# temudschin/xfemm

Measured on AMD Instinct MI355X. Metric: solved DoF/s (assembly+CG to tol) on 2M-tri magnetostatic, higher is better.
Workload: dtype f64; 1 GPU; configs[2]: synthetic 2000000-tri square-domain magnetostatic, linear mu, tol 1e-08; triangles=2000000, dof_total=1002001, dof_per_gpu=1002001, nnz=7006001, pcg_iters=18, newton_iters=1, pcg=Chronopoulos-Gear + AMG V-cycle, parallelism=single GPU

## Files before the change

### include/xfemm_kernels.h

```cpp
#ifndef XFEMM_KERNELS_H
#define XFEMM_KERNELS_H

#ifdef __cplusplus
extern "C" {
#endif

enum {
    XFK_OK = 0,
    XFK_ERR_ARG = -1,
    XFK_ERR_HIP = -2,
    XFK_ERR_SINGULAR = -3,
    XFK_ERR_NOCONV = -4,
    XFK_ERR_UNSUPPORTED = -5
};

typedef struct {
    double mu_x, mu_y;
    double H_c;
    double J_re;
    double Cduct;
    double LamFill;
    int LamType;
    int BHpoints;
    const double *B;
// ... 386 lines not shown
typedef struct {
    int sweeps;
    double theta, omega;
    int dense_max, fold, col16, f32, wlevel;
} xfk_amg_probe_opts;
typedef struct {
    int n, nc, fold, has16, has32, w_at;
    long long nnz, pnnz, fnnz;
    double weight, rho_f;
} xfk_amg_level_info;
typedef struct {
    int levels, dense_coarse, cinv_f64, traced;
    xfk_amg_level_info level[16];
} xfk_amg_info;
enum { XFK_AMG_A = 0, XFK_AMG_P = 1, XFK_AMG_R = 2, XFK_AMG_PF = 3, XFK_AMG_RF = 4,
       XFK_AMG_PLAIN_COLS = 16, XFK_AMG_F64_VALS = 32 };
enum { XFK_AMG_DINV = 0, XFK_AMG_DENSE = 1 };
enum { XFK_AMG_TR_SFLAG = 0, XFK_AMG_TR_SDEG = 1, XFK_AMG_TR_AGG = 2, XFK_AMG_TR_AGG_PRE = 3,
       XFK_AMG_TR_ROOT = 4, XFK_AMG_TR_DFINV = 5, XFK_AMG_TR_WF = 6 };
int xfk_amg_probe_create(int n, const int *rowptr, const int *col, const double *val, int device,
                         const xfk_amg_probe_opts *opts, int trace, xfk_amg_probe **out);
int xfk_amg_probe_info(xfk_amg_probe *probe, xfk_amg_info *info);
int xfk_amg_probe_level_size(xfk_amg_probe *probe, int level, int sel, int *rows, int *cols, long long *nnz);
int xfk_amg_probe_level_csr(xfk_amg_probe *probe, int level, int sel, int *rowptr, int *col, double *val);
int xfk_amg_probe_tiles(xfk_amg_probe *probe, int sel, int *tiles, int *wide);
int xfk_amg_probe_vector(xfk_amg_probe *probe, int level, int what, double *out);
int xfk_amg_probe_trace(xfk_amg_probe *probe, int level, int what, void *out);
int xfk_amg_probe_apply(xfk_amg_probe *probe, int nvec, const double *R, double *U);
int xfk_amg_probe_refresh(xfk_amg_probe *probe, const double *val, int fold);
void xfk_amg_probe_destroy(xfk_amg_probe *probe);

int xfk_get_csr(xfk_problem *prob, int *rowptr, int *col, double *val, double *b);
long long xfk_get_nnz(xfk_problem *prob);
double xfk_spmv_col_bytes(xfk_problem *prob);
int xfk_get_stream(xfk_problem *prob, void **hip_stream);

int xfk_pcg_solve_csr(int n, const int *rowptr, const int *col, const double *val,
                      const double *b, double *V, int flag, double precision,
                      int device, long long *iters, double *er);
int xfk_pcg_solve_csr_pc(int n, const int *rowptr, const int *col, const double *val,
                         const double *b, double *V, int flag, double precision,
                         int device, int precond, long long *iters, double *er);

int xfk_age_element_matrix(double ci, double co, double K, double Ki, double *MG);

int xfk_pcg_time(xfk_problem *prob, int iters, double *ms_spmv, double *ms_iter);

typedef struct {
    char name[64];
    int calls;
    double ms_total;
    double bytes_per_call;
} xfk_phase;
enum { XFK_PROFILE_SETUP = 1 };
int xfk_phase_profile(xfk_problem *prob, int iters, int flags, xfk_phase *out, int cap, int *count);

int xfk_alloc_stats(double *out4, int reset);

int xfk_problem_memory(const xfk_problem *prob, long long *out4);
int xfk_cache_stats(long long *out3);
int xfk_release_cache(void);

int xfk_amg_forget_hints(void);

int xfk_sort_elements(int n_elems, const unsigned *score, int device, int *perm);

// ... 14 lines not shown
```

### xfemm_amd/csrc/xfk_api.hip

```cpp
#include <hipcub/hipcub.hpp>

#include "xfk_amg.h"
#include "xfk_spmv.h"

#include <algorithm>
#include <atomic>
#include <chrono>
#include <cmath>
#include <cstring>
#include <map>
#include <mutex>
#include <iterator>
#include <set>
#include <type_traits>
#include <unordered_map>

#include "xfk_age.h"
#include "xfk_comm.h"
#include "xfk_kernels.h"
#include "xfk_magdir.h"
#include <cstdio>
#include <cstdlib>
#include "xfk_partition.h"

// ... 722 lines not shown
    launch_row_build(s, N, P->p_raw.p, P->n2e_ptr.p, P->n2e.p, fp, fc, T.rowtmp, T.rowcnt, P->n2e.p);
    XFK_CHECK(exclusive_scan(P, T.rowcnt, P->rowptr.p, N));
    XFK_CHECK(hipMemcpyAsync(P->hpin, P->rowptr.p + N, sizeof(int), hipMemcpyDeviceToHost, s));
    XFK_CHECK(hipMemcpyAsync(P->hpin + 1, P->rowptr.p + P->N, sizeof(int), hipMemcpyDeviceToHost, s));
    P->hpin[5] = 0;
    if (!P->harmonic && N > 0 && P->amg && P->amg->cap_hint.empty()) {
        void *tmp = nullptr;
        size_t bytes = 0;
        XFK_CHECK(hipcub::DeviceReduce::Max(tmp, bytes, T.rowcnt, T.cnt + 3, N, s));
        XFK_CHECK(cub_scratch(P, bytes, &tmp));
        XFK_CHECK(hipcub::DeviceReduce::Max(tmp, bytes, T.rowcnt, T.cnt + 3, N, s));
        XFK_CHECK(hipMemcpyAsync(P->hpin + 5, T.cnt + 3, sizeof(int), hipMemcpyDeviceToHost, s));
    }
    const long long bound_nnz = 6LL * NE + N + nfill;
    const bool defer = !P->harmonic && P->age_key.empty() && P->pbc_entry_key.empty() &&
                       bound_nnz * 12 <= (512LL << 20);
    long long cap_nnz;
    if (defer) {
        if (!P->nnz_ev) XFK_CHECK(hipEventCreateWithFlags(&P->nnz_ev, hipEventDisableTiming));
        XFK_CHECK(hipEventRecord(P->nnz_ev, s));
        P->nnz_pending = true;
        cap_nnz = bound_nnz;
    } else {
        XFK_CHECK(hipStreamSynchronize(s));
        P->nnz = P->hpin[0];
        P->nnz_own = P->hpin[1];
        P->row_max = P->hpin[5];
        P->nnz_pending = false;
        cap_nnz = P->nnz;
    }
    XFK_CHECK(P->col.alloc(cap_nnz));
    XFK_CHECK(P->val.alloc(cap_nnz));
    XFK_CHECK(P->diag.alloc(N));
    launch_row_copy(s, N, P->p_raw.p, P->n2e_ptr.p, P->n2e.p, fp, fc, T.rowtmp, P->rowptr.p, P->col.p, P->diag.p);

    P->ncolors = 0;
    P->color_rounds = 0;
    if (P->harmonic) {
    XFK_CHECK(P->color.alloc(NE));
    XFK_CHECK(hipMemsetAsync(P->color.p, 0xff, sizeof(int) * NE, s));
    constexpr int kSyncRounds = 6;
    XFK_CHECK(hipMemsetAsync(T.active, 1, (size_t)NL, s));
    int round = 0, last = 0;
    for (;;) {
        XFK_REQUIRE(round < SymTmp::kMaxRounds, XFK_ERR_UNSUPPORTED, "element colouring did not terminate");
        for (int k = 0; k < kSyncRounds; ++k, ++round)
            launch_jp_round(s, NL, NE, round, T.active, T.cnt + 2, P->p_raw.p, P->n2e_ptr.p, P->n2e.p, P->color.p,
                            T.maxkey, T.used);
        XFK_CHECK(d2h(&last, T.cnt + 2, sizeof(int), s));
        if (last < round) break;
    }
    round = last + 1;
    P->color_rounds = round;
    const int maxc = SymTmp::kMaxColors;
    launch_color_hist(s, NE, P->color.p, T.hist, maxc);
    std::vector<int> hh(maxc + 1);
    XFK_CHECK(d2h(hh.data(), T.hist, sizeof(int) * (maxc + 1), s));
    XFK_REQUIRE(hh[maxc] == 0, XFK_ERR_UNSUPPORTED, "more than 128 element colours needed");
    int nc = 0;
    for (int c = 0; c < maxc; ++c)
        if (hh[c]) nc = c + 1;
    P->ncolors = nc;
    P->color_off.assign(nc + 1, 0);
    for (int c = 0; c < nc; ++c) P->color_off[c + 1] = P->color_off[c] + hh[c];

    XFK_CHECK(P->perm.alloc(NE));
    launch_iota(s, NE, T.iota);
    {
        void *tmp = nullptr;
        size_t bytes = 0;
        XFK_CHECK(hipcub::DeviceRadixSort::SortPairs(tmp, bytes, P->color.p, T.keys_out, T.iota, P->perm.p, NE, 0,
                                                     8, s));
        XFK_CHECK(cub_scratch(P, bytes, &tmp));
        XFK_CHECK(hipcub::DeviceRadixSort::SortPairs(tmp, bytes, P->color.p, T.keys_out, T.iota, P->perm.p, NE, 0,
                                                     8, s));
    }
    XFK_CHECK(P->erec.alloc(NE));
    XFK_CHECK(P->ebits.alloc(NE));
    XFK_CHECK(P->slot.alloc(9 * (size_t)NE));
    launch_build_erec(s, NE, P->perm.p, P->p_raw.p, P->lbl_raw.p, P->ebits_raw.p, P->erec.p, P->ebits.p, T.iperm);
    launch_build_slots(s, NE, N, P->p_raw.p, T.iperm, P->rowptr.p, P->col.p, P->slot.p, T.cnt);
    }

    launch_mark_fix_adj(s, N, P->rowptr.p, P->col.p, P->fixed.p, T.flag);
    XFK_CHECK(P->fix_cols_row.alloc(N));
    launch_compact_flags(s, N, T.flag, T.cnt + 1, P->fix_cols_row.p);
    if (P->harmonic) {
        XFK_CHECK(hipMemcpyAsync(P->hpin + 2, T.cnt, sizeof(int) * 2, hipMemcpyDeviceToHost, s));
        XFK_CHECK(hipStreamSynchronize(s));
        const int hc[2] = {P->hpin[2], P->hpin[3]};
        XFK_REQUIRE(hc[0] == 0, XFK_ERR_HIP, "internal: element slot missing from the CSR pattern");
        P->nfix_cols = hc[1];
    } else {
        XFK_CHECK(P->nfix_dev.alloc(1));
        XFK_CHECK(hipMemcpyAsync(P->nfix_dev.p, T.cnt + 1, sizeof(int), hipMemcpyDeviceToDevice, s));
        P->nfix_cols = -1;
    }
    XFK_CHECK(P->mu1.alloc(NE));
    XFK_CHECK(P->mu2.alloc(NE));
    if (!P->harmonic) {
        XFK_CHECK(P->mu1b.alloc(NE));
        XFK_CHECK(P->mu2b.alloc(NE));
        if (P->any_nonlinear && !P->axi) {
            XFK_CHECK(P->dv_el.alloc(NE));
            XFK_CHECK(P->on_el.alloc(NE));
        }
        XFK_CHECK(P->asm_miss.alloc(1));
        XFK_CHECK(hipMemsetAsync(P->asm_miss.p, 0, sizeof(int), s));
        P->miss_checked = false;
    }

    P->age_n = 0;
    if (!P->age_key.empty()) {
        std::vector<int> rc;
        std::vector<double> v;
        for (size_t m = 0; m < P->age_key.size(); ++m) {
            const int r = (int)(P->age_key[m] >> 32), c = (int)(P->age_key[m] & 0xffffffff);
            rc.push_back(r); rc.push_back(c); v.push_back(P->age_val[m]);
            if (r != c) { rc.push_back(c); rc.push_back(r); v.push_back(P->age_val[m]); }
        }
        const int na = (int)v.size();
        DBuf<int> d_rc;
        XFK_CHECK(upload(d_rc, rc.data(), rc.size(), s));
        XFK_CHECK(upload(P->age_v, v.data(), v.size(), s));
        XFK_CHECK(P->age_slot.alloc(na));
        launch_lookup_slots(s, na, d_rc.p, P->rowptr.p, P->col.p, P->age_slot.p);
        std::vector<int> chk(na);
        XFK_CHECK(d2h(chk.data(), P->age_slot.p, sizeof(int) * na, s));
// ... 127 lines not shown
    A.blocks = P->blocks.p;
    A.lines = P->lines.p;
    A.circs = P->circs.p;
    A.bhB = P->bhB.p;
    A.bhH = P->bhH.p;
    A.bhS = P->bhS.p;
    A.mu1 = P->mu1.p;
    A.mu2 = P->mu2.p;
    A.V = P->V.p;
    A.val = P->val.p;
    A.b = P->b.p;
    A.iter = iter;
    A.axi = P->axi ? 1 : 0;
    A.ext_ro = P->ext_ro;
    A.ext_ri = P->ext_ri;
    A.ext_zo = P->ext_zo;
    A.p_raw = P->p_raw.p;
    A.lbl_raw = P->lbl_raw.p;
    A.ebits_raw = P->ebits_raw.p;
    A.n2e_ptr = P->n2e_ptr.p;
    A.n2e = P->n2e.p;
    A.rowptr = P->rowptr.p;
    A.col = P->col.p;
    A.mu1_out = P->any_nonlinear ? P->mu1b.p : nullptr;
    A.mu2_out = P->any_nonlinear ? P->mu2b.p : nullptr;
    A.miss = P->asm_miss.p;
    const bool pre = P->any_nonlinear && !P->axi && P->dv_el.p && env_int("XFK_ASM_STATE", 1) != 0;
    A.dv_el = pre ? P->dv_el.p : nullptr;
    A.on_el = pre ? P->on_el.p : nullptr;
    A.n_el = P->NE;
    if (P->electro) launch_electro_rows(s, P);
    else if (P->heat) launch_heat_rows(s, P);
    else if (P->mask) launch_mask_rows(s, P);
    else launch_assemble_rows(s, P->NR, A);
    std::swap(P->mu1.p, P->mu1b.p);
    std::swap(P->mu1.n, P->mu1b.n);
    std::swap(P->mu2.p, P->mu2b.p);
    std::swap(P->mu2.n, P->mu2b.n);
    launch_add_at_slots(s, P->age_n, P->age_slot.p, P->age_v.p, P->val.p);
    launch_point_currents(s, P->npt, P->pt_nodes.p, P->pt_J.p, P->b.p);
    launch_dirichlet(s, P->nfix_rows, P->fix_rows.p, P->nfix_cols, P->nfix_dev.p, P->N, P->fix_cols_row.p,
                     P->rowptr.p, P->col.p, P->diag.p, P->fixed.p, P->fix_first.p, P->fix_last.p, P->val.p, P->b.p);
    launch_map(s, P->pm_n, P->pm_dst.p, P->pm_ptr.p, P->pm_src.p, P->pm_w.p, P->val.p, P->pm_tmp.p);
    launch_map(s, P->pb_n, P->pb_dst.p, P->pb_ptr.p, P->pb_src.p, P->pb_w.p, P->b.p, P->pb_tmp.p);
    XFK_CHECK(hipGetLastError());
    return XFK_OK;
}

static int alloc_cg(xfk_problem *P)
{
    const int N = P->N, NL = P->NL;
    int G = std::max(cg_grid(N), cg_axpy_grid(N));
    if (P->comm)
        for (int q = 0; q < P->nranks; ++q) {
            const int nq = (int)(row_begin(P->N_global, q + 1, P->nranks) - row_begin(P->N_global, q, P->nranks));
            G = std::max(G, std::max(cg_grid(nq), cg_axpy_grid(nq)));
        }
    P->Gpart = G;
    XFK_CHECK(P->R2.alloc((size_t)N));
    XFK_CHECK(P->W2.alloc((size_t)N));
    XFK_CHECK(P->Z2.alloc((size_t)N + NL));
    XFK_CHECK(P->part_loc.alloc(4 * (size_t)G));
    if (P->comm) {
        XFK_CHECK(P->part_glob_buf.alloc(4 * (size_t)G));
        P->part_glob = P->part_glob_buf.p;
    } else {
// ... 1530 lines not shown
    return XFK_OK;
}

long long xfk_get_nnz(xfk_problem *P) { return P && xfk_resolve_nnz(P) == XFK_OK ? P->nnz_own : -1; }

double xfk_spmv_col_bytes(xfk_problem *P)
{
    if (!P || xfk_resolve_nnz(P) != XFK_OK) return -1.0;
    const unsigned short *c16;
    const int *cbase;
    spmv_col16(P, c16, cbase);
    if (!c16 || P->nnz_own <= 0) return 4.0;
    const int N = P->N, nt = (N + kCgBlock - 1) / kCgBlock;
    std::vector<int> base(nt), rp(N + 1);
    if (d2h(base.data(), cbase, sizeof(int) * nt, P->stream) != hipSuccess ||
        d2h(rp.data(), P->rowptr.p, sizeof(int) * (N + 1), P->stream) != hipSuccess)
        return -1.0;
    long long wide = 0;
    for (int t = 0; t < nt; ++t)
        if (base[t] == kNoColBase) wide += rp[std::min(N, (t + 1) * kCgBlock)] - rp[t * kCgBlock];
    return (2.0 * (double)P->nnz_own + 2.0 * (double)wide) / (double)P->nnz_own;
}

int xfk_get_csr(xfk_problem *P, int *rowptr, int *col, double *val, double *b)
{
    XFK_REQUIRE(P && P->symbolic_ready, XFK_ERR_ARG, "no assembled system");
    XFK_CHECK(hipSetDevice(P->device));
    XFK_CHECK(hipStreamSynchronize(P->stream));
    if (xfk_resolve_nnz(P) != XFK_OK) return XFK_ERR_HIP;
    if (rowptr) XFK_CHECK(d2h(rowptr, P->rowptr.p, sizeof(int) * (P->N + 1), P->stream));
    if (col) XFK_CHECK(d2h(col, P->col.p, sizeof(int) * P->nnz_own, P->stream));
    if (val) XFK_CHECK(d2h(val, P->val.p, sizeof(double) * P->nnz_own, P->stream));
    if (b) XFK_CHECK(d2h(b, P->b.p, sizeof(double) * P->N, P->stream));
    return XFK_OK;
}

int xfk_get_stream(xfk_problem *P, void **st)
{
    XFK_REQUIRE(P && st, XFK_ERR_ARG, "null argument");
    *st = (void *)P->stream;
    return XFK_OK;
}

int xfk_pcg_solve_csr(int n, const int *rowptr, const int *col, const double *val, const double *b, double *V,
                      int flag, double precision, int device, long long *iters, double *er)
{
    return xfk_pcg_solve_csr_pc(n, rowptr, col, val, b, V, flag, precision, device, XFK_PRECOND_JACOBI, iters, er);
}

int xfk_set_option(xfk_problem *P, int option, double value)
{
    XFK_REQUIRE(P, XFK_ERR_ARG, "null problem");
    switch (option) {
    case XFK_OPT_PRECOND:
        XFK_REQUIRE(value == XFK_PRECOND_JACOBI || value == XFK_PRECOND_AMG, XFK_ERR_ARG, "unknown preconditioner");
        P->precond = (int)value;
        return XFK_OK;
    case XFK_OPT_AMG_SWEEPS:
        XFK_REQUIRE(value >= 1 && value <= 8 && value == (int)value, XFK_ERR_ARG, "AMG sweeps must be 1..8");
        P->amg_sweeps = (int)value;
        return XFK_OK;
    case XFK_OPT_AMG_THETA:
        XFK_REQUIRE(value >= 0.0 && value < 1.0, XFK_ERR_ARG, "AMG strength threshold must be in [0, 1)");
        P->amg_theta = value;
        return XFK_OK;
    case XFK_OPT_AMG_OMEGA:
// ... 360 lines not shown
```

### xfemm_amd/csrc/xfk_device.hip

```cpp
#include "xfk_kernels.h"
#include "xfk_axi.h"
#include "xfk_spmv.h"

namespace xfk {


__device__ __forceinline__ double wave_sum(double v)
{
#pragma unroll
    for (int off = 32; off > 0; off >>= 1) v += __shfl_xor(v, off, 64);
    return v;
}

__device__ __forceinline__ double block_sum(double v, double *lds)
{
    v = wave_sum(v);
    const int lane = threadIdx.x & 63, wid = threadIdx.x >> 6;
    __syncthreads();
    if (lane == 0) lds[wid] = v;
    __syncthreads();
    double r = 0.0;
    if (threadIdx.x == 0) {
        const int nw = (blockDim.x + 63) >> 6;
        for (int w = 0; w < nw; ++w) r += lds[w];
// ... 799 lines not shown
            double Km = 0.0001 * bp.H_c * (lab.cos_m * (X[k] - X[j]) + lab.sin_m * (Y[k] - Y[j])) / 2.;
            be[j] += Km;
            be[k] += Km;
        }
    }

    const double Vn[3] = {A.V[n[0]], A.V[n[1]], A.V[n[2]]};
    if (FIRST) {
        const double f = bp.LamFill;
        if (bp.LamType == 0) { m1 = bp.mu_x * f + (1. - f); m2 = bp.mu_y * f + (1. - f); }
        else if (bp.LamType == 1) { m1 = bp.mu_x * f + (1. - f); m2 = bp.mu_x / (f + bp.mu_x * (1. - f)); }
        else if (bp.LamType == 2) { m2 = bp.mu_y * f + (1. - f); m1 = bp.mu_y / (f + bp.mu_y * (1. - f)); }
        else { m1 = 1; m2 = 1; }
    } else {
        double dv = pre_dv;
        const bool on = PRE ? pre_on : planar_newton_state(A, bp, p, q, a, Vn, m1, m2, dv);
        if (on) planar_newton_terms(bp, Mx, My, a, Vn, dv, Mn);
    }

    const double im1 = 1.0 / m1, im2 = 1.0 / m2;
#pragma unroll
    for (int j = 0; j < 3; ++j)
#pragma unroll
        for (int k = 0; k < 3; ++k) {
            Me[j][k] += (Mx[j][k] * im2 + My[j][k] * im1 + Mn[j][k]);
            be[j] += Mn[j][k] * Vn[k];
        }

}

constexpr int kRowBlock = 128;
constexpr int kRowAcc = 12;

template <bool AXI, bool FIRST, bool PRE>
__device__ __forceinline__ void assemble_rows(int N, const AssembleArgs &A)
{
    __shared__ double s_acc[kRowAcc * kRowBlock];
    __shared__ int s_col[kRowAcc * kRowBlock];
    const int i0 = xcd_tile(blockIdx.x, gridDim.x) * kRowBlock;
    const int i = i0 + threadIdx.x;
    const bool live = i < N;
    const int rs = live ? A.rowptr[i] : 0, L = live ? A.rowptr[i + 1] - rs : 0;
    const bool lds = L <= kRowAcc;
    double *acc = lds ? s_acc + threadIdx.x : A.val + rs;
    const int stride = lds ? kRowBlock : 1;
    const int *cols = lds ? s_col + threadIdx.x : A.col + rs;
    for (int k = 0; k < L; ++k) {
        acc[k * stride] = 0.;
        if (lds) s_col[k * kRowBlock + threadIdx.x] = A.col[rs + k];
    }
    double bi = 0.;
    bool miss = false;
    const int t1 = live ? A.n2e_ptr[i + 1] : 0;
    for (int t = live ? A.n2e_ptr[i] : 0; t < t1; ++t) {
        const int e = A.n2e[t];
        const int n[3] = {A.p_raw[3 * e], A.p_raw[3 * e + 1], A.p_raw[3 * e + 2]};
        const int j = (n[0] == i) ? 0 : ((n[1] == i) ? 1 : 2);
        const DevLabel lab = A.labels[A.lbl_raw[e]];
        const DevBlock bp = A.blocks[lab.blk];
        const double X[3] = {A.x[n[0]], A.x[n[1]], A.x[n[2]]};
        const double Y[3] = {A.y[n[0]], A.y[n[1]], A.y[n[2]]};
        double m1 = 0., m2 = 0., Me[3][3], be[3];
        if (PRE) {
            m1 = A.mu1_out[e];
            m2 = A.mu2_out[e];
        } else if (!FIRST) {
            m1 = A.mu1[e];
            m2 = A.mu2[e];
        }
        if (AXI) axi_element<FIRST>(A.ebits_raw[e], A, n, X, Y, lab, bp, m1, m2, Me, be);
        else if (PRE) planar_element<false, true>(A.ebits_raw[e], A, n, X, Y, lab, bp, m1, m2, Me, be, A.dv_el[e], A.on_el[e] != 0);
        else planar_element<FIRST>(A.ebits_raw[e], A, n, X, Y, lab, bp, m1, m2, Me, be);
        const int w = (n[0] < N) ? 0 : ((n[1] < N) ? 1 : 2);
        if (!PRE && w == j && A.mu1_out) {
            A.mu1_out[e] = m1;
            A.mu2_out[e] = m2;
        }
#pragma unroll
        for (int k = 0; k < 3; ++k) {
            const double m = (j == 0) ? Me[0][k] : ((j == 1) ? ((k >= 1) ? Me[1][k] : Me[0][1])
                                                             : ((k == 2) ? Me[2][2] : Me[k][2]));
            int pos = 0;
            while (pos < L - 1 && cols[pos * stride] != n[k]) ++pos;
            miss |= cols[pos * stride] != n[k];
            acc[pos * stride] -= m;
        }
        bi -= (j == 0) ? be[0] : ((j == 1) ? be[1] : be[2]);
    }
    if (miss && A.miss) *A.miss = 1;
    if (__syncthreads_and(lds)) {
        double r[kRowAcc];
#pragma unroll
        for (int k = 0; k < kRowAcc; ++k) r[k] = k < L ? s_acc[k * kRowBlock + threadIdx.x] : 0.;
        const int rb0 = A.rowptr[i0], rb1 = A.rowptr[min(i0 + kRowBlock, N)];
        __syncthreads();
#pragma unroll
        for (int k = 0; k < kRowAcc; ++k)
            if (k < L) s_acc[rs - rb0 + k] = r[k];
        __syncthreads();
        for (int m = threadIdx.x; m < rb1 - rb0; m += kRowBlock) A.val[rb0 + m] = s_acc[m];
    } else if (lds) {
        for (int k = 0; k < L; ++k) A.val[rs + k] = s_acc[k * kRowBlock + threadIdx.x];
    }
    if (live) A.b[i] = bi;
}

template <bool AXI, bool FIRST>
__global__ void __launch_bounds__(kRowBlock) k_assemble_rows(int N, AssembleArgs A)
{
    assemble_rows<AXI, FIRST, false>(N, A);
}

__global__ void __launch_bounds__(kRowBlock, 4) k_assemble_rows_pre(int N, AssembleArgs A)
{
    assemble_rows<false, false, true>(N, A);
}

__global__ void __launch_bounds__(256) k_planar_state(int NE, AssembleArgs A)
{
    const int e = blockIdx.x * blockDim.x + threadIdx.x;
    if (e >= NE) return;
    const DevLabel lab = A.labels[A.lbl_raw[e]];
    const DevBlock bp = A.blocks[lab.blk];
    double m1 = A.mu1[e], m2 = A.mu2[e], dv = 0;
    bool on = false;
    if (bp.BHpoints > 0 && bp.LamType <= 2 && (bp.LamType != 0 || m1 == m2)) {
        const int n[3] = {A.p_raw[3 * e], A.p_raw[3 * e + 1], A.p_raw[3 * e + 2]};
        const double X[3] = {A.x[n[0]], A.x[n[1]], A.x[n[2]]};
        const double Y[3] = {A.y[n[0]], A.y[n[1]], A.y[n[2]]};
        const double Vn[3] = {A.V[n[0]], A.V[n[1]], A.V[n[2]]};
        double p[3], q[3];
        const double a = planar_geometry(X, Y, p, q);
        on = planar_newton_state(A, bp, p, q, a, Vn, m1, m2, dv);
    }
    A.mu1_out[e] = m1;
    A.mu2_out[e] = m2;
    A.dv_el[e] = dv;
    A.on_el[e] = on ? 1 : 0;
}

__global__ void k_point_currents(int n, const int *__restrict__ nodes, const double *__restrict__ J,
                                 double *__restrict__ b)
{
    int i = blockIdx.x * blockDim.x + threadIdx.x;
    if (i < n) b[nodes[i]] += J[i];
// ... 208 lines not shown
}
void launch_lookup_slots(hipStream_t s, int n, const int *rc, const int *rowptr, const int *col, int *out)
{
    if (n) k_lookup_slots<<<nblk(n), kBlock, 0, s>>>(n, rc, rowptr, col, out);
}
void launch_mark_fix_adj(hipStream_t s, int N, const int *rowptr, const int *col, const unsigned char *fixed,
                         int *flag)
{
    if (N) k_mark_fix_adj<<<nblk(N), kBlock, 0, s>>>(N, rowptr, col, fixed, flag);
}
void launch_compact_flags(hipStream_t s, int N, const int *flag, int *cursor, int *out)
{
    if (N) k_compact_flags<<<nblk(N), kBlock, 0, s>>>(N, flag, cursor, out);
}
void launch_assemble_rows(hipStream_t s, int N, const AssembleArgs &A)
{
    if (N <= 0) return;
    const int g = (N + kRowBlock - 1) / kRowBlock;
    if (A.axi) {
        if (A.iter == 0) k_assemble_rows<true, true><<<g, kRowBlock, 0, s>>>(N, A);
        else k_assemble_rows<true, false><<<g, kRowBlock, 0, s>>>(N, A);
    } else {
        if (A.iter == 0) {
            k_assemble_rows<false, true><<<g, kRowBlock, 0, s>>>(N, A);
        } else if (A.dv_el && A.mu1_out) {
            if (A.n_el > 0) k_planar_state<<<(A.n_el + 255) / 256, 256, 0, s>>>(A.n_el, A);
            k_assemble_rows_pre<<<g, kRowBlock, 0, s>>>(N, A);
        } else {
            k_assemble_rows<false, false><<<g, kRowBlock, 0, s>>>(N, A);
        }
    }
}

void launch_point_currents(hipStream_t s, int n, const int *nodes, const double *J, double *b)
{
    if (n) k_point_currents<<<nblk(n), kBlock, 0, s>>>(n, nodes, J, b);
}
void launch_dirichlet(hipStream_t s, int nrows, const int *rows, int nadj, const int *nadj_dev, int nadj_max,
                      const int *adj, const int *rowptr, const int *col, const int *diag, const unsigned char *fixed,
                      const double *fix_first, const double *fix_last, double *val, double *b)
{
    if (nadj < 0) {
        if (nadj_max > 0)
            k_dirichlet_cols_d<<<std::min(nblk(nadj_max), 1024), kBlock, 0, s>>>(nadj_dev, adj, rowptr, col, fixed,
                                                                              fix_first, val, b);
    } else if (nadj) {
        k_dirichlet_cols<<<nblk(nadj), kBlock, 0, s>>>(nadj, adj, rowptr, col, fixed, fix_first, val, b);
    }
    if (nrows) k_dirichlet_rows<<<nblk(nrows), kBlock, 0, s>>>(nrows, rows, rowptr, diag, val, b, fix_last);
}
void launch_add_at_slots(hipStream_t s, int n, const int *slot, const double *v, double *data)
{
    if (n) k_add_at_slots<<<nblk(n), kBlock, 0, s>>>(n, slot, v, data);
}
void launch_map(hipStream_t s, int n, const int *dst, const int *ptr, const int *src, const double *w,
                double *data, double *tmp)
{
    if (!n) return;
    k_map_gather<<<nblk(n), kBlock, 0, s>>>(n, ptr, src, w, data, tmp);
    k_map_scatter<<<nblk(n), kBlock, 0, s>>>(n, dst, tmp, data);
}
void launch_diag_inv(hipStream_t s, int N, const int *diag, const double *val, double *dinv, CgState *S)
{
    if (N) k_diag_inv<<<nblk(N), kBlock, 0, s>>>(N, diag, val, dinv, S);
}
void launch_newton_res(hipStream_t s, int N, const double *V, const double *Vold, double *partials,
// ... 21 lines not shown
```

### xfemm_amd/csrc/xfk_internal.h

```cpp
#pragma once

#include <hip/hip_runtime.h>

#include <algorithm>
#include <chrono>
#include <cstdint>
#include <cstdlib>
#include <map>
#include <string>
#include <unordered_map>
#include <thread>
#include <vector>

#include "../../include/xfemm_kernels.h"
#include "xfk_partition.h"

struct xfk_comm;

namespace xfk {

struct Amg;

constexpr int kBlock = 256;
constexpr int kRedGrid = 1024;
// ... 314 lines not shown
    double precision = 1e-8, relax = 1.0;
    bool any_nonlinear = false;

    xfk::DBuf<double> x, y;
    xfk::DBuf<int> p_raw;
    xfk::DBuf<int> lbl_raw;
    xfk::DBuf<int> ebits_raw;

    xfk::DBuf<xfk::DevBlock> blocks;
    xfk::DBuf<xfk::DevLabel> labels;
    xfk::DBuf<xfk::DevLine> lines;
    xfk::DBuf<xfk::DevCirc> circs;
    xfk::DBuf<double> bhB, bhH, bhS;
    int nblocks = 0, nlabels = 0, nlines = 0, ncircs = 0;

    bool symbolic_ready = false;
    xfk::DBuf<int> n2e_ptr, n2e;
    xfk::DBuf<int> rowptr, col, diag;
    xfk::DBuf<int> color;
    int color_rounds = 0;
    xfk::DBuf<char> cub_tmp;
    xfk::DBuf<char> sym_tmp;
    xfk::DBuf<int> fill_ptr, fill_col;
    xfk::DBuf<int> perm;
    xfk::DBuf<int4> erec;
    xfk::DBuf<int> ebits;
    xfk::DBuf<int> slot;
    xfk::DBuf<double> mu1, mu2;
    xfk::DBuf<double> mu1b, mu2b;
    xfk::DBuf<double> dv_el;
    xfk::DBuf<unsigned char> on_el;
    xfk::DBuf<int> asm_miss;
    bool miss_checked = false;

    xfk::DBuf<int> pt_nodes;
    xfk::DBuf<double> pt_J;
    int npt = 0;
    xfk::DBuf<unsigned char> fixed;
    xfk::DBuf<double> fix_first, fix_last;
    xfk::DBuf<int> fix_rows;
    int nfix_rows = 0;
    xfk::DBuf<int> fix_cols;
    xfk::DBuf<int> fix_cols_node;
    xfk::DBuf<int> fix_cols_row;
    int nfix_cols = 0;
    xfk::DBuf<int> nfix_dev;
    xfk::DBuf<int> pm_dst, pm_ptr, pm_src;
    xfk::DBuf<double> pm_w, pm_tmp;
    int pm_n = 0;
    xfk::DBuf<int> pb_dst, pb_ptr, pb_src;
    xfk::DBuf<double> pb_w, pb_tmp;
    int pb_n = 0;
    std::vector<long long> pbc_fill;
    std::vector<long long> age_key;
    std::vector<double> age_val;
    xfk::DBuf<int> age_slot;
    xfk::DBuf<double> age_v;
    int age_n = 0;
    std::vector<std::pair<long long, double>> pbc_entry_terms;
    std::vector<int> pbc_entry_ptr;
    std::vector<long long> pbc_entry_key;
    std::vector<std::pair<int, double>> pbc_b_terms;
    std::vector<int> pbc_b_ptr;
    std::vector<int> pbc_b_key;
    std::vector<std::pair<long long, double>> pbca_entry_terms;
    std::vector<int> pbca_entry_ptr;
// ... 283 lines not shown
```

### xfemm_amd/csrc/xfk_kernels.h

```cpp
#pragma once

#include "xfk_internal.h"

namespace xfk {

struct AssembleArgs {
    const int4 *erec;
    const int *ebits;
    const int *slot;
    const double *x, *y;
    const DevLabel *labels;
    const DevBlock *blocks;
    const DevLine *lines;
    const DevCirc *circs;
    const double *bhB, *bhH, *bhS;
    double *mu1, *mu2;
    const double *V;
    double *val, *b;
    int iter;
    int axi;
    double ext_ro, ext_ri, ext_zo;
    const int *p_raw, *lbl_raw, *ebits_raw, *n2e_ptr, *n2e, *rowptr, *col;
    double *mu1_out, *mu2_out;
    int *miss;
    double *dv_el;
    unsigned char *on_el;
    int n_el;
};

int grid_reduce(int N);

struct CgAxpyArgs {
    const double *W, *dinv;
    double *Z, *P, *V, *R, *U;
    const double *gam_in;
    const double *del_in;
    const double *reso;
    double *gam_out;
    int Ggam, Gdel;
    CgState *S;
    long long it;
    int N;
    int amg;
};

int cg_grid(int N);
int cg_axpy_grid(int N);
void launch_cg_init_r(hipStream_t s, int N, int flag, const int *rowptr, const int *col, const double *val,
                      const double *b, double *V, double *R, double *U, double *Z, double *P, const double *dinv,
                      double *part_reso, double *part_gam0);
void launch_cg_axpy(hipStream_t s, const CgAxpyArgs &A);
void launch_cg_spmv(hipStream_t s, int N, const int *rowptr, const int *col, const double *val, const double *U,
                    double *W, double *part_del, const CgState *S, const double *R = nullptr,
                    double *part_gam = nullptr, const int *tiles = nullptr, int ntiles = 0,
                    const unsigned short *c16 = nullptr, const int *cbase = nullptr);
void launch_cg_dot(hipStream_t s, int N, const double *a, const double *b, double *part);
void launch_cg_state_init(hipStream_t s, CgState *S, double tol, double tol_rel = 0.0);

void launch_count_incidence(hipStream_t s, int NE, const int *p, int *deg);
void launch_fill_n2e(hipStream_t s, int NE, const int *p, const int *ptr, int *cursor, int *n2e);
void launch_sort_segments(hipStream_t s, int N, const int *ptr, int *a);
void launch_n2e_count(hipStream_t s, int NE, const int *p, int *deg);
void launch_n2e_fill(hipStream_t s, int NE, const int *p, const int *ptr, int *cursor, int *n2e);
void launch_n2e_sort(hipStream_t s, int v0, int NL, const int *ptr, int *n2e);
long long row_tmp_size(int N, int NE, int nfill);
void launch_row_build(hipStream_t s, int N, const int *p, const int *n2e_ptr, const int *n2e, const int *fill_ptr,
                      const int *fill_col, int *tmp, int *rowcnt,
                      int *n2e_sort = nullptr);
void launch_row_copy(hipStream_t s, int N, const int *p, const int *n2e_ptr, const int *n2e, const int *fill_ptr,
                     const int *fill_col, const int *tmp, const int *rowptr, int *col, int *diag);
void launch_jp_round(hipStream_t s, int N, int NE, int round, unsigned char *active, int *pending_round,
                     const int *p, const int *n2e_ptr, const int *n2e, int *color, unsigned long long *maxkey,
                     unsigned long long *used);
void launch_color_hist(hipStream_t s, int NE, const int *color, int *hist, int maxc);
void launch_iota(hipStream_t s, int n, int *a);
void launch_build_erec(hipStream_t s, int NE, const int *perm, const int *p, const int *lbl, const int *ebits_raw,
                       int4 *erec, int *ebits, int *iperm);
void launch_build_slots(hipStream_t s, int NE, int nrows, const int *p, const int *iperm, const int *rowptr,
                        const int *col, int *slot, int *bad);
void launch_add_at_slots(hipStream_t s, int n, const int *slot, const double *v, double *data);
void launch_lookup_slots(hipStream_t s, int n, const int *rc, const int *rowptr, const int *col, int *out);
void launch_mark_fix_adj(hipStream_t s, int N, const int *rowptr, const int *col, const unsigned char *fixed,
                         int *flag);
void launch_compact_flags(hipStream_t s, int N, const int *flag, int *cursor, int *out);
void launch_assemble_rows(hipStream_t s, int N, const AssembleArgs &A);
void launch_point_currents(hipStream_t s, int n, const int *nodes, const double *J, double *b);
void launch_dirichlet(hipStream_t s, int nrows, const int *rows, int nadj, const int *nadj_dev, int nadj_max,
                      const int *adj, const int *rowptr, const int *col, const int *diag, const unsigned char *fixed,
                      const double *fix_first, const double *fix_last, double *val, double *b);
void launch_map(hipStream_t s, int n, const int *dst, const int *ptr, const int *src, const double *w,
                double *data, double *tmp);
void launch_diag_inv(hipStream_t s, int N, const int *diag, const double *val, double *dinv, CgState *S);
void launch_newton_res(hipStream_t s, int N, const double *V, const double *Vold, double *partials,
                       unsigned *counter, NewtonScalars *S);
void launch_relax(hipStream_t s, int N, double relax, double *V, const double *Vold);
void launch_scale(hipStream_t s, int N, double sc, const double *V, double *out);

}
```

### xfemm_amd/kernels.py

```python
from __future__ import annotations

import ctypes as C
import cmath
import math
import os
from typing import Optional, Sequence

import numpy as np

HERE = os.path.dirname(os.path.abspath(__file__))
LIB_DIR = os.path.join(HERE, "lib")
KERNELS_SO = os.path.join(LIB_DIR, "libxfemm_kernels.so")

dptr = C.POINTER(C.c_double)
iptr = C.POINTER(C.c_int)

XFK_OK = 0
XFK_REBUILD_SYMBOLIC = 1
XFK_TIME_SPMV = 2
XFK_TIME_TAIL = 4
XFK_PRECOND_JACOBI = 0
XFK_PRECOND_AMG = 1
PRECONDS = {"jacobi": XFK_PRECOND_JACOBI, "amg": XFK_PRECOND_AMG}
XFK_OPT_PRECOND = 1
XFK_OPT_AMG_SWEEPS = 2
XFK_OPT_AMG_THETA = 3
XFK_OPT_AMG_OMEGA = 4
XFK_OPT_AMG_REPLICATE = 5
XFK_OPT_AMG_REUSE = 6
XFK_OPT_AMG_DENSE = 7
XFK_OPT_AMG_FOLD = 8
XFK_OPT_AMG_COL16 = 9
XFK_OPT_AMG_WLEVEL = 10
XFK_OPT_AMG_F32 = 11
XFK_OPT_NEWTON_INEXACT = 12
XFK_OPT_HEAT_MAX_PASSES = 13

EXPORTED = (
    "xfk_last_error", "xfk_age_element_matrix", "xfk_device_count", "xfk_device_init", "xfk_problem_create", "xfk_problem_destroy",
    "xfk_static2d", "xfk_get_solution", "xfk_get_circuits", "xfk_get_csr", "xfk_get_nnz", "xfk_spmv_col_bytes",
    "xfk_get_stream", "xfk_pcg_solve_csr", "xfk_pcg_solve_csr_pc", "xfk_pcg_time", "xfk_phase_profile",
    "xfk_alloc_stats", "xfk_problem_memory", "xfk_cache_stats", "xfk_release_cache",
    "xfk_amg_forget_hints",
    "xfk_set_option",
    "xfk_problem_create_harmonic", "xfk_problem_create_harmonic_dist", "xfk_harmonic2d",
    "xfk_get_solution_complex", "xfk_get_circuits_complex",
    "xfk_get_csr_complex",
    "xfk_comm_unique_id", "xfk_comm_create_rccl", "xfk_comm_create_local", "xfk_comm_destroy",
    "xfk_comm_rank", "xfk_comm_size", "xfk_comm_record", "xfk_comm_log", "xfk_comm_create_replay",
    "xfk_comm_time", "xfk_comm_timing",
    "xfk_partition_plan", "xfk_partition_plan_coupled", "xfk_problem_create_dist", "xfk_dist_get_info",
    "xfk_magdir_eval", "xfk_magdir_eval_labels", "xfk_lua_run", "xfk_sort_elements",
    "xfk_problem_create_electrostatic", "xfk_electrostatic", "xfk_get_conductors", "xfk_conductor_charge",
    "xfk_problem_create_heatflow", "xfk_heatflow", "xfk_heatflow_assemble", "xfk_heatflow_set_step",
    "xfk_heatflow_advance", "xfk_hf_get_conductors", "xfk_hf_conductor_flow",
    "xfk_pot_set_solution", "xfk_pot_get_qmarks", "xfk_pot_set_qmarks", "xfk_pot_plot_bounds", "xfk_pot_block_integrals_ordered",
    "xfk_pot_point_values_at", "xfk_pot_element_fields", "xfk_pot_corner_fields", "xfk_pot_corner_branches",
    "xfk_pot_block_integrals", "xfk_pot_block_integral", "xfk_pot_point_values", "xfk_pot_grid_info", "xfk_pot_time",
    "xfk_pot_make_mask", "xfk_pot_get_mask", "xfk_pot_mask_info", "xfk_pot_mask_problem", "xfk_pot_stress_time",
    "xfk_pot_line_integrals", "xfk_pot_line_integral", "xfk_pot_contour_samples", "xfk_pot_contour_time",
    "xfk_mag_set_solution", "xfk_mag_set_depth", "xfk_mag_element_b", "xfk_mag_block_integrals",
    "xfk_mag_block_integral", "xfk_mag_time",
    "xfk_mag_ac_set_solution", "xfk_mag_ac_element_b", "xfk_mag_ac_block_integrals", "xfk_mag_ac_block_integral",
    "xfk_mag_ac_time",
    "xfk_mag_make_mask", "xfk_mag_get_mask", "xfk_mag_mask_info", "xfk_mag_mask_problem", "xfk_mag_stress_time",
    "xfk_mag_corner_b", "xfk_mag_point_values", "xfk_mag_point_values_at", "xfk_mag_line_integrals",
    "xfk_mag_line_integral", "xfk_mag_contour_samples", "xfk_mag_point_time", "xfk_mag_contour_time",
    "xfk_amg_probe_create", "xfk_amg_probe_info", "xfk_amg_probe_level_size", "xfk_amg_probe_level_csr",
    "xfk_amg_probe_tiles", "xfk_amg_probe_vector", "xfk_amg_probe_trace", "xfk_amg_probe_apply",
    "xfk_amg_probe_refresh", "xfk_amg_probe_destroy",
)


# ... 149 lines not shown
                ("w_at", C.c_int), ("nnz", C.c_longlong), ("pnnz", C.c_longlong), ("fnnz", C.c_longlong),
                ("weight", C.c_double), ("rho_f", C.c_double)]


class AmgInfo(C.Structure):
    _fields_ = [("levels", C.c_int), ("dense_coarse", C.c_int), ("cinv_f64", C.c_int), ("traced", C.c_int),
                ("level", AmgLevelInfo * 16)]


_lib = None


class XfkError(RuntimeError):
    pass


def load_library(path: str = KERNELS_SO):
    global _lib
    if _lib is not None:
        return _lib
    if not os.path.exists(path):
        raise XfkError("HIP library %s not built (run __graft_entry__.build() / make -C xfemm_amd)" % path)
    L = C.CDLL(path)
    L.xfk_last_error.restype = C.c_char_p
    L.xfk_device_count.restype = C.c_int
    L.xfk_problem_create.argtypes = [C.POINTER(ProblemDesc), C.c_int, C.POINTER(C.c_void_p)]
    L.xfk_problem_destroy.argtypes = [C.c_void_p]
    L.xfk_static2d.argtypes = [C.c_void_p, C.c_int, C.POINTER(Result)]
    L.xfk_get_solution.argtypes = [C.c_void_p, dptr]
    L.xfk_get_circuits.argtypes = [C.c_void_p, iptr, dptr, dptr]
    L.xfk_get_csr.argtypes = [C.c_void_p, iptr, iptr, dptr, dptr]
    L.xfk_get_nnz.argtypes = [C.c_void_p]
    L.xfk_get_nnz.restype = C.c_longlong
    L.xfk_spmv_col_bytes.argtypes = [C.c_void_p]
    L.xfk_spmv_col_bytes.restype = C.c_double
    L.xfk_get_stream.argtypes = [C.c_void_p, C.POINTER(C.c_void_p)]
    L.xfk_pcg_solve_csr.argtypes = [C.c_int, iptr, iptr, dptr, dptr, dptr, C.c_int, C.c_double, C.c_int,
                                    C.POINTER(C.c_longlong), dptr]
    L.xfk_pcg_solve_csr_pc.argtypes = [C.c_int, iptr, iptr, dptr, dptr, dptr, C.c_int, C.c_double, C.c_int,
                                       C.c_int, C.POINTER(C.c_longlong), dptr]
    L.xfk_pcg_time.argtypes = [C.c_void_p, C.c_int, dptr, dptr]
    L.xfk_amg_probe_create.argtypes = [C.c_int, iptr, iptr, dptr, C.c_int, C.POINTER(AmgProbeOpts), C.c_int,
                                       C.POINTER(C.c_void_p)]
    L.xfk_amg_probe_info.argtypes = [C.c_void_p, C.POINTER(AmgInfo)]
    L.xfk_amg_probe_level_size.argtypes = [C.c_void_p, C.c_int, C.c_int, iptr, iptr, C.POINTER(C.c_longlong)]
    L.xfk_amg_probe_level_csr.argtypes = [C.c_void_p, C.c_int, C.c_int, iptr, iptr, dptr]
    L.xfk_amg_probe_tiles.argtypes = [C.c_void_p, C.c_int, iptr, iptr]
    L.xfk_amg_probe_vector.argtypes = [C.c_void_p, C.c_int, C.c_int, dptr]
    L.xfk_amg_probe_trace.argtypes = [C.c_void_p, C.c_int, C.c_int, C.c_void_p]
    L.xfk_amg_probe_apply.argtypes = [C.c_void_p, C.c_int, dptr, dptr]
    L.xfk_amg_probe_refresh.argtypes = [C.c_void_p, dptr, C.c_int]
    L.xfk_amg_probe_destroy.argtypes = [C.c_void_p]
    L.xfk_amg_probe_destroy.restype = None
    L.xfk_phase_profile.argtypes = [C.c_void_p, C.c_int, C.c_int, C.c_void_p, C.c_int, C.POINTER(C.c_int)]
    L.xfk_alloc_stats.argtypes = [dptr, C.c_int]
    L.xfk_problem_memory.argtypes = [C.c_void_p, C.POINTER(C.c_longlong)]
    L.xfk_cache_stats.argtypes = [C.POINTER(C.c_longlong)]
    L.xfk_set_option.argtypes = [C.c_void_p, C.c_int, C.c_double]
    L.xfk_problem_create_harmonic.argtypes = [C.POINTER(ProblemDesc), C.c_void_p, C.c_int, C.POINTER(C.c_void_p)]
    L.xfk_problem_create_harmonic_dist.argtypes = [C.POINTER(ProblemDesc), C.c_void_p, C.c_int, C.c_void_p,
                                                   C.POINTER(C.c_void_p)]
    L.xfk_harmonic2d.argtypes = [C.c_void_p, C.c_int, C.POINTER(Result)]
    L.xfk_get_solution_complex.argtypes = [C.c_void_p, dptr]
    L.xfk_get_circuits_complex.argtypes = [C.c_void_p, iptr, dptr, dptr]
    L.xfk_get_csr_complex.argtypes = [C.c_void_p, iptr, iptr, dptr, dptr]
    L.xfk_age_element_matrix.argtypes = [C.c_double, C.c_double, C.c_double, C.c_double, dptr]
# ... 596 lines not shown
        flags = ((XFK_REBUILD_SYMBOLIC if rebuild_symbolic else 0) | (XFK_TIME_SPMV if time_spmv else 0) |
                 (XFK_TIME_TAIL if time_tail else 0))
        _check(_lib.xfk_static2d(self._h, flags, C.byref(r)))
        self.result = r
        return r.as_dict()

    def solution(self) -> np.ndarray:
        A = np.zeros(self.n_nodes)
        _check(_lib.xfk_get_solution(self._h, A.ctypes.data_as(dptr)))
        return A

    def circuits(self):
        n = self.n_circs
        cc = np.zeros(max(1, n), np.int32)
        J = np.zeros(max(1, n))
        dV = np.zeros(max(1, n))
        _check(_lib.xfk_get_circuits(self._h, cc.ctypes.data_as(iptr), J.ctypes.data_as(dptr),
                                     dV.ctypes.data_as(dptr)))
        return cc[:n], J[:n], dV[:n]

    def spmv_col_bytes(self) -> float:
        return float(_lib.xfk_spmv_col_bytes(self._h))

    def csr(self):
        nnz = _lib.xfk_get_nnz(self._h)
        rp = np.zeros(self.n_rows + 1, np.int32)
        col = np.zeros(nnz, np.int32)
        val = np.zeros(nnz)
        b = np.zeros(self.n_rows)
        _check(_lib.xfk_get_csr(self._h, rp.ctypes.data_as(iptr), col.ctypes.data_as(iptr),
                                val.ctypes.data_as(dptr), b.ctypes.data_as(dptr)))
        return rp, col, val, b

    def pcg_time(self, iters: int = 50):
        ms_spmv = C.c_double()
        ms_iter = C.c_double()
        _check(_lib.xfk_pcg_time(self._h, iters, C.byref(ms_spmv), C.byref(ms_iter)))
        return ms_spmv.value, ms_iter.value

    def phase_profile(self, iters: int = 10, setup: bool = True):
        cap = 256
        buf = (Phase * cap)()
        n = C.c_int()
        _check(_lib.xfk_phase_profile(self._h, iters, XFK_PROFILE_SETUP if setup else 0, C.cast(buf, C.c_void_p),
                                      cap, C.byref(n)))
        out = []
        for k in range(n.value):
            ph = buf[k]
            out.append(dict(name=ph.name.decode(), calls=ph.calls, ms_total=ph.ms_total,
                            us_per_call=1e3 * ph.ms_total / max(1, ph.calls), bytes_per_call=ph.bytes_per_call))
        return out


class Contour:

    def __init__(self, points=()):
        self.points = []
        for x, y in points:
            self.add(x, y)

    def __len__(self):
        return len(self.points)

    def add(self, x, y):
        z = (float(x), float(y))
        if not self.points or z != self.points[-1]:
# ... 944 lines not shown
```

Baseline: 192.6 million DoF/s.

## Fuse CSR column fill and fixed-adjacency marking into first assembly pass

For plain magnetostatic problems, the separate row-copy kernel and the mark/compact of fixed-adjacent rows are deferred. The first assembly launch now does that work inside a row-pass variant, writing column indices, diagonal positions and fixed-adjacency entries while it builds values. This removes two or three setup kernels and one extra pass over the column array. In exchange, the first assembly gets more complex, and fixed-adjacency order now comes from atomics rather than a compaction. A debug accessor is also added.

```diff
diff --git a/include/xfemm_kernels.h b/include/xfemm_kernels.h
--- a/include/xfemm_kernels.h
+++ b/include/xfemm_kernels.h
@@ -442,6 +442,7 @@
 
 int xfk_get_csr(xfk_problem *prob, int *rowptr, int *col, double *val, double *b);
 long long xfk_get_nnz(xfk_problem *prob);
+int xfk_get_pattern_aux(xfk_problem *prob, int *diag, int *fix_adj, int *n_fix_adj);
 double xfk_spmv_col_bytes(xfk_problem *prob);
 int xfk_get_stream(xfk_problem *prob, void **hip_stream);
 
diff --git a/xfemm_amd/csrc/xfk_api.hip b/xfemm_amd/csrc/xfk_api.hip
--- a/xfemm_amd/csrc/xfk_api.hip
+++ b/xfemm_amd/csrc/xfk_api.hip
@@ -778,7 +778,13 @@
     XFK_CHECK(P->col.alloc(cap_nnz));
     XFK_CHECK(P->val.alloc(cap_nnz));
     XFK_CHECK(P->diag.alloc(N));
-    launch_row_copy(s, N, P->p_raw.p, P->n2e_ptr.p, P->n2e.p, fp, fc, T.rowtmp, P->rowptr.p, P->col.p, P->diag.p);
+    const bool rowpass = !P->harmonic && !P->electro && !P->heat && !P->mask && !P->comm && fillv.empty() &&
+                         P->age_key.empty() && P->pbc_entry_key.empty();
+    P->rowpass_pending = rowpass;
+    P->rowpass_tmp = T.rowtmp;
+    P->rowpass_count = T.cnt + 1;
+    if (!rowpass)
+        launch_row_copy(s, N, P->p_raw.p, P->n2e_ptr.p, P->n2e.p, fp, fc, T.rowtmp, P->rowptr.p, P->col.p, P->diag.p);
 
     P->ncolors = 0;
     P->color_rounds = 0;
@@ -828,9 +834,11 @@
     launch_build_slots(s, NE, N, P->p_raw.p, T.iperm, P->rowptr.p, P->col.p, P->slot.p, T.cnt);
     }
 
-    launch_mark_fix_adj(s, N, P->rowptr.p, P->col.p, P->fixed.p, T.flag);
     XFK_CHECK(P->fix_cols_row.alloc(N));
-    launch_compact_flags(s, N, T.flag, T.cnt + 1, P->fix_cols_row.p);
+    if (!rowpass) {
+        launch_mark_fix_adj(s, N, P->rowptr.p, P->col.p, P->fixed.p, T.flag);
+        launch_compact_flags(s, N, T.flag, T.cnt + 1, P->fix_cols_row.p);
+    }
     if (P->harmonic) {
         XFK_CHECK(hipMemcpyAsync(P->hpin + 2, T.cnt, sizeof(int) * 2, hipMemcpyDeviceToHost, s));
         XFK_CHECK(hipStreamSynchronize(s));
@@ -839,7 +847,8 @@
         P->nfix_cols = hc[1];
     } else {
         XFK_CHECK(P->nfix_dev.alloc(1));
-        XFK_CHECK(hipMemcpyAsync(P->nfix_dev.p, T.cnt + 1, sizeof(int), hipMemcpyDeviceToDevice, s));
+        if (!rowpass)
+            XFK_CHECK(hipMemcpyAsync(P->nfix_dev.p, T.cnt + 1, sizeof(int), hipMemcpyDeviceToDevice, s));
         P->nfix_cols = -1;
     }
     XFK_CHECK(P->mu1.alloc(NE));
@@ -1033,6 +1042,13 @@
     if (P->electro) launch_electro_rows(s, P);
     else if (P->heat) launch_heat_rows(s, P);
     else if (P->mask) launch_mask_rows(s, P);
+    else if (P->rowpass_pending) {
+        XFK_REQUIRE(iter == 0, XFK_ERR_HIP, "internal: the CSR pattern is not filled yet");
+        const RowPassArgs R = {P->rowpass_tmp, P->col.p, P->diag.p, P->fixed.p, P->fix_cols_row.p, P->rowpass_count};
+        launch_assemble_rowpass(s, P->NR, A, R);
+        XFK_CHECK(hipMemcpyAsync(P->nfix_dev.p, P->rowpass_count, sizeof(int), hipMemcpyDeviceToDevice, s));
+        P->rowpass_pending = false;
+    }
     else launch_assemble_rows(s, P->NR, A);
     std::swap(P->mu1.p, P->mu1b.p);
     std::swap(P->mu1.n, P->mu1b.n);
@@ -2629,6 +2645,18 @@
     if (col) XFK_CHECK(d2h(col, P->col.p, sizeof(int) * P->nnz_own, P->stream));
     if (val) XFK_CHECK(d2h(val, P->val.p, sizeof(double) * P->nnz_own, P->stream));
     if (b) XFK_CHECK(d2h(b, P->b.p, sizeof(double) * P->N, P->stream));
+    return XFK_OK;
+}
+
+int xfk_get_pattern_aux(xfk_problem *P, int *diag, int *fix_adj, int *n_fix_adj)
+{
+    XFK_REQUIRE(P && P->symbolic_ready && !P->rowpass_pending, XFK_ERR_ARG, "no assembled system");
+    XFK_CHECK(hipSetDevice(P->device));
+    int n = P->nfix_cols;
+    if (n < 0) XFK_CHECK(d2h(&n, P->nfix_dev.p, sizeof(int), P->stream));
+    if (diag) XFK_CHECK(d2h(diag, P->diag.p, sizeof(int) * P->N, P->stream));
+    if (fix_adj && n > 0) XFK_CHECK(d2h(fix_adj, P->fix_cols_row.p, sizeof(int) * n, P->stream));
+    if (n_fix_adj) *n_fix_adj = n;
     return XFK_OK;
 }
 
diff --git a/xfemm_amd/csrc/xfk_device.hip b/xfemm_amd/csrc/xfk_device.hip
--- a/xfemm_amd/csrc/xfk_device.hip
+++ b/xfemm_amd/csrc/xfk_device.hip
@@ -855,8 +855,50 @@
 constexpr int kRowBlock = 128;
 constexpr int kRowAcc = 12;
 
-template <bool AXI, bool FIRST, bool PRE>
-__device__ __forceinline__ void assemble_rows(int N, const AssembleArgs &A)
+template <int W>
+__device__ __forceinline__ int rowpass_regs(int i, int s, int ne, const RowCands &rc, int rs, const RowPassArgs &R,
+                                            int *s_c)
+{
+    int a[W];
+    row_regs<W>(i, s, ne, rc, a);
+    int u = 0, f = 0;
+#pragma unroll
+    for (int q = 0; q < W; ++q)
+        if (a[q] != INT_MAX && (q == 0 || a[q] != a[q - 1])) {
+            R.col[rs + u] = a[q];
+            if (s_c) s_c[u * kRowBlock] = a[q];
+            if (a[q] == i) R.diag[i] = rs + u;
+            f |= R.fixed[a[q]];
+            ++u;
+        }
+    return f;
+}
+
+__device__ __forceinline__ void rowpass_pattern(int i, int rs, int L, const AssembleArgs &A, const RowPassArgs &R,
+                                                int *s_c)
+{
+    const RowCands rc{A.p_raw, A.n2e_ptr, A.n2e, nullptr, nullptr};
+    const int s = A.n2e_ptr[i], ne = A.n2e_ptr[i + 1] - s;
+    int f = 0;
+    if (ne <= 7) {
+        f = rowpass_regs<16>(i, s, ne, rc, rs, R, s_c);
+    } else if (ne <= kRowRegElems) {
+        f = rowpass_regs<32>(i, s, ne, rc, rs, R, s_c);
+    } else {
+        const int *src = R.tmp + rc.base(i);
+        for (int k = 0; k < L; ++k) {
+            const int c = src[k];
+            R.col[rs + k] = c;
+            if (s_c) s_c[k * kRowBlock] = c;
+            if (c == i) R.diag[i] = rs + k;
+            f |= R.fixed[c];
+        }
+    }
+    if (f && !R.fixed[i]) R.fix_adj[atomicAdd(R.fix_count, 1)] = i;
+}
+
+template <bool AXI, bool FIRST, bool PRE, bool ROWPASS = false>
+__device__ __forceinline__ void assemble_rows(int N, const AssembleArgs &A, const RowPassArgs &R = RowPassArgs{})
 {
     __shared__ double s_acc[kRowAcc * kRowBlock];
     __shared__ int s_col[kRowAcc * kRowBlock];
@@ -868,9 +910,10 @@
     double *acc = lds ? s_acc + threadIdx.x : A.val + rs;
     const int stride = lds ? kRowBlock : 1;
     const int *cols = lds ? s_col + threadIdx.x : A.col + rs;
+    if (ROWPASS && live) rowpass_pattern(i, rs, L, A, R, lds ? s_col + threadIdx.x : nullptr);
     for (int k = 0; k < L; ++k) {
         acc[k * stride] = 0.;
-        if (lds) s_col[k * kRowBlock + threadIdx.x] = A.col[rs + k];
+        if (!ROWPASS && lds) s_col[k * kRowBlock + threadIdx.x] = A.col[rs + k];
     }
     double bi = 0.;
     bool miss = false;
@@ -934,6 +977,12 @@
     assemble_rows<AXI, FIRST, false>(N, A);
 }
 
+template <bool AXI>
+__global__ void __launch_bounds__(kRowBlock) k_assemble_rowpass(int N, AssembleArgs A, RowPassArgs R)
+{
+    assemble_rows<AXI, true, false, true>(N, A, R);
+}
+
 __global__ void __launch_bounds__(kRowBlock, 4) k_assemble_rows_pre(int N, AssembleArgs A)
 {
     assemble_rows<false, false, true>(N, A);
@@ -1208,6 +1257,14 @@
     }
 }
 
+void launch_assemble_rowpass(hipStream_t s, int N, const AssembleArgs &A, const RowPassArgs &R)
+{
+    if (N <= 0) return;
+    const int g = (N + kRowBlock - 1) / kRowBlock;
+    if (A.axi) k_assemble_rowpass<true><<<g, kRowBlock, 0, s>>>(N, A, R);
+    else k_assemble_rowpass<false><<<g, kRowBlock, 0, s>>>(N, A, R);
+}
+
 void launch_point_currents(hipStream_t s, int n, const int *nodes, const double *J, double *b)
 {
     if (n) k_point_currents<<<nblk(n), kBlock, 0, s>>>(n, nodes, J, b);
diff --git a/xfemm_amd/csrc/xfk_internal.h b/xfemm_amd/csrc/xfk_internal.h
--- a/xfemm_amd/csrc/xfk_internal.h
+++ b/xfemm_amd/csrc/xfk_internal.h
@@ -370,6 +370,9 @@
     xfk::DBuf<unsigned char> on_el;
     xfk::DBuf<int> asm_miss;
     bool miss_checked = false;
+    bool rowpass_pending = false;
+    const int *rowpass_tmp = nullptr;
+    int *rowpass_count = nullptr;
 
     xfk::DBuf<int> pt_nodes;
     xfk::DBuf<double> pt_J;
diff --git a/xfemm_amd/csrc/xfk_kernels.h b/xfemm_amd/csrc/xfk_kernels.h
--- a/xfemm_amd/csrc/xfk_kernels.h
+++ b/xfemm_amd/csrc/xfk_kernels.h
@@ -26,6 +26,13 @@
     double *dv_el;
     unsigned char *on_el;
     int n_el;
+};
+
+struct RowPassArgs {
+    const int *tmp;
+    int *col, *diag;
+    const unsigned char *fixed;
+    int *fix_adj, *fix_count;
 };
 
 int grid_reduce(int N);
@@ -84,6 +91,7 @@
                          int *flag);
 void launch_compact_flags(hipStream_t s, int N, const int *flag, int *cursor, int *out);
 void launch_assemble_rows(hipStream_t s, int N, const AssembleArgs &A);
+void launch_assemble_rowpass(hipStream_t s, int N, const AssembleArgs &A, const RowPassArgs &R);
 void launch_point_currents(hipStream_t s, int n, const int *nodes, const double *J, double *b);
 void launch_dirichlet(hipStream_t s, int nrows, const int *rows, int nadj, const int *nadj_dev, int nadj_max,
                       const int *adj, const int *rowptr, const int *col, const int *diag, const unsigned char *fixed,
diff --git a/xfemm_amd/kernels.py b/xfemm_amd/kernels.py
--- a/xfemm_amd/kernels.py
+++ b/xfemm_amd/kernels.py
@@ -38,7 +38,7 @@
 
 EXPORTED = (
     "xfk_last_error", "xfk_age_element_matrix", "xfk_device_count", "xfk_device_init", "xfk_problem_create", "xfk_problem_destroy",
-    "xfk_static2d", "xfk_get_solution", "xfk_get_circuits", "xfk_get_csr", "xfk_get_nnz", "xfk_spmv_col_bytes",
+    "xfk_static2d", "xfk_get_solution", "xfk_get_circuits", "xfk_get_csr", "xfk_get_nnz", "xfk_get_pattern_aux", "xfk_spmv_col_bytes",
     "xfk_get_stream", "xfk_pcg_solve_csr", "xfk_pcg_solve_csr_pc", "xfk_pcg_time", "xfk_phase_profile",
     "xfk_alloc_stats", "xfk_problem_memory", "xfk_cache_stats", "xfk_release_cache",
     "xfk_amg_forget_hints",
@@ -254,6 +254,7 @@
     L.xfk_get_csr.argtypes = [C.c_void_p, iptr, iptr, dptr, dptr]
     L.xfk_get_nnz.argtypes = [C.c_void_p]
     L.xfk_get_nnz.restype = C.c_longlong
+    L.xfk_get_pattern_aux.argtypes = [C.c_void_p, iptr, iptr, C.POINTER(C.c_int)]
     L.xfk_spmv_col_bytes.argtypes = [C.c_void_p]
     L.xfk_spmv_col_bytes.restype = C.c_double
     L.xfk_get_stream.argtypes = [C.c_void_p, C.POINTER(C.c_void_p)]
@@ -916,6 +917,13 @@
                                 val.ctypes.data_as(dptr), b.ctypes.data_as(dptr)))
         return rp, col, val, b
 
+    def pattern_aux(self):
+        diag = np.zeros(self.n_rows, np.int32)
+        adj = np.zeros(max(1, self.n_rows), np.int32)
+        n = C.c_int()
+        _check(_lib.xfk_get_pattern_aux(self._h, diag.ctypes.data_as(iptr), adj.ctypes.data_as(iptr), C.byref(n)))
+        return diag, np.sort(adj[:n.value])
+
     def pcg_time(self, iters: int = 50):
         ms_spmv = C.c_double()
         ms_iter = C.c_double()
```

New measurement: 194.1 million DoF/s, median of 6. Within noise of the previous version (+0.8%).
